# junliu111/CV-MonoSLAM

Hardware: AMD Instinct MI355X
Metric: srukf_updates_per_sec (higher is better)
Workload: dtype f64; 1 GPU; BASELINE configs[2]: 200 inverse-depth landmarks (n=1204, Na=1209, L=2419), M=N matched, fp64, one batched refactor per frame, synthetic 640x480 figure-8 sequence; landmarks=200, state_dim=1204, sequences_per_gpu=1, update_mode=batched

## Files before the change

### cv-monoslam_amd/csrc/srukf_batch.hip

```cpp

#include "srukf_ctx.h"
using namespace srukf_impl;

struct BatchPlan {
    std::vector<srukf_ctx*> cs;
    int B = 0;
    Pxy2Args* t_pxy2 = nullptr; GainArgs* t_gain = nullptr; SyrkArgs* t_syrk = nullptr; SyrkOwnArgs* t_own = nullptr; Step64Args* t_step = nullptr; ExpandArgs* t_exp = nullptr;
    hipGraph_t g1 = nullptr, g8 = nullptr; hipGraphExec_t e1 = nullptr, e8 = nullptr;
    std::vector<unsigned long long> sig;
};
struct BatchDev { BatchPlan* plans[SRUKF_BATCH_GROUPS_MAX] = {}; hipStream_t streams[SRUKF_BATCH_GROUPS_MAX] = {}; };
static thread_local std::map<int, BatchDev> g_batch_dev;
static hipStream_t batch_stream(int device, int grp)
{
    BatchDev& bd = g_batch_dev[device];
    if (!bd.streams[0]) {
        if (hipSetDevice(device) != hipSuccess) return nullptr;
        for (int q = 0; q < SRUKF_BATCH_GROUPS_MAX; q++) if (hipStreamCreateWithFlags(&bd.streams[q], hipStreamNonBlocking) != hipSuccess) bd.streams[q] = nullptr;
    }
    return bd.streams[grp];
}
static void batch_plan_drop_graphs(BatchPlan* bp)
{
    if (bp->e1) { hipGraphExecDestroy(bp->e1); bp->e1 = nullptr; }
// ... 42 lines not shown
    for (auto& kv : g_batch_dev)
        for (int grp = 0; grp < SRUKF_BATCH_GROUPS_MAX; grp++) if (kv.second.plans[grp]) { hipSetDevice(kv.first); hipStreamSynchronize(kv.second.streams[grp]); batch_plan_drop_graphs(kv.second.plans[grp]); }
}
}
static bool batch_eligible(srukf_ctx* const* cs, int B, bool ignore_canonical = false)
{
    if (B < 2 || B > 64 || !g_dbg_batch_wide.load()) return false;
    const srukf_ctx* a = cs[0];
    for (int b = 0; b < B; b++) {
        const srukf_ctx* c = cs[b];
        for (int q = 0; q < b; q++) if (cs[q] == c) return false;
        if (c->device != a->device || c->d.N != a->d.N || c->d.N < 1 || c->storage != SRUKF_STORAGE_F64 || c->w.wc0 != c->w.wm0) return false;
        if (c->red_r <= 0 || c->red_r != a->red_r || c->red_Tp != a->red_Tp || !c->shadowA || (!c->null_canonical && !ignore_canonical) || !c->nskip || !c->tail_ok) return false;
        if (c->ns_full != a->ns_full || c->ns_null != a->ns_null || c->ns_rows != a->ns_rows || c->n_pxy2_tiles != a->n_pxy2_tiles) return false;
        if (c->n_syrk_head_tiles != a->n_syrk_head_tiles || c->gplan_red.ntiles != a->gplan_red.ntiles || c->pxy2_split_b0 != a->pxy2_split_b0 || memcmp(&c->w, &a->w, sizeof c->w) != 0) return false;
        if (!c->dbg.pxy2 || !c->dbg.nullskip || !c->dbg.tail_fuse || c->dbg.fused_motion != 2 || !c->dbg.table_perm || c->profiling || c->use_graph != a->use_graph || c->debug_starve) return false;
        if (memcmp(&c->p, &a->p, sizeof c->p) != 0 || c->gplan_red.T < 16 || (size_t)c->d.np * sizeof(double) > 48 * 1024 || !rank_fused_mode()) return false;
        if (!c->odo_seq || c->seqF != a->seqF) return false;
    }
    return true;
}
static void batch_frame(const BatchPlan* bp, hipStream_t st)
{
    const srukf_ctx* c = bp->cs[0];
    const KDims& d = c->d;
    const int n = d.n, np = d.np, r = c->red_r, Tp = c->red_Tp, B = bp->B, kr = (r + 15) & ~15;
    srukf_launch_pxy2_b(st, d, bp->t_pxy2, B, c->pxy2_tiles, c->n_pxy2_tiles, kr, c->w, (d.N + 31) / 32);
    srukf_launch_gain_b(st, d, c->w, bp->t_gain, B, c->pxy2_split_b0, sqrt(c->p.epsilon));
    srukf_launch_syrk_b(st, d, bp->t_syrk, B, g_dbg_batch_xcd.load() ? c->syrk_head_tiles_b : c->syrk_head_tiles, g_dbg_batch_xcd.load() ? c->n_syrk_head_tiles_b : c->n_syrk_head_tiles, std::min(np, kr), (n + 255) / 256,
                        (n - r + SRUKF_RANK_COLS - 1) / SRUKF_RANK_COLS);
    srukf_launch_syrk_own_b(st, n, np, bp->t_own, B, 0, d.mp, kr, c->gplan_red.tiles, c->gplan_red.ntiles, Tp);
    int pb = 0;
    for (int j0 = -64; j0 + 64 < np && j0 + 64 <= 64 * Tp; j0 += 64, pb ^= 1) {
        if (!g_dbg_batch_split.load()) {
            srukf_launch_gmw_step64_b(st, n, np, j0, c->p.epsilon, bp->t_step, B, std::max(1, Tp - j0 / 64 - 1), pb);
            continue;
        }
        const int rows = Tp - j0 / 64 - 1, pair = j0 >= 0 ? (j0 / 64) & 1 : 0;
        const bool k128 = g_dbg_batch_k128.load() != 0;
        const bool first_of_pair = k128 && j0 >= 0 && pair == 0 && rows - 1 >= 1 && j0 + 128 < np && j0 + 128 <= 64 * Tp;
        const bool second_of_pair = k128 && j0 >= 64 && pair == 1 && rows >= 1;
        srukf_launch_gmw_pivslab_b(st, n, np, j0, c->p.epsilon, bp->t_step, B, pb, second_of_pair ? 1 : 0);
        if (j0 >= 0 && rows >= 1) srukf_launch_gmw_trail_b(st, np, j0, bp->t_step, B, rows, second_of_pair ? 1 : 0, first_of_pair ? 1 : second_of_pair ? 2 : 0);
    }
    srukf_launch_rank_expand_b(st, n, np, r, c->p.epsilon, bp->t_exp, B, c->w.gamma, d, c->w, c->p);
}
static int batch_capture(BatchPlan* bp, hipStream_t st, int nframes, hipGraph_t* g, hipGraphExec_t* ge)
{
    srukf_ctx* c = bp->cs[0];
    HIPCHK(c, hipStreamBeginCapture(st, hipStreamCaptureModeThreadLocal));
    for (int q = 0; q < nframes; q++) batch_frame(bp, st);
    const hipError_t launch_err = hipGetLastError();
    HIPCHK(c, hipStreamEndCapture(st, g));
    HIPCHK(c, launch_err);
    HIPCHK(c, hipGraphInstantiate(ge, *g, nullptr, nullptr, 0));
    return SRUKF_OK;
}
static int batch_run(srukf_ctx* const* cs, int B, int first, int count, double* const* dt, int grp)
{
    srukf_ctx* c0 = cs[0];
// ... 178 lines not shown
```

### cv-monoslam_amd/csrc/srukf_ctx.h

```cpp
#pragma once
#include <hip/hip_runtime.h>
#include <math.h>
#include <stdio.h>
#include <stdlib.h>
#include <string.h>
#include <string>
#include <cstddef>
#include <vector>
#include <algorithm>
#include <utility>
#include <atomic>
#include <mutex>
#include <map>
#include "srukf_launch.h"

#define SRUKF_GRAPH_FRAMES 8
#define SRUKF_MAX_TENANTS 4
#define SRUKF_NULL_ENERGY 1e-12
#ifndef SRUKF_BATCH_GROUPS_MAX
#define SRUKF_BATCH_GROUPS_MAX 4
#endif

enum KClass { KC_MOTION = 0, KC_PROJECT, KC_STATS, KC_PXY, KC_GAIN, KC_SYRK, KC_GMW_TRAIL, KC_GMW_PERSIST, KC_GMW_CHECK,
              KC_GMW_COL, KC_RANK_EXPAND, KC_PROJECT_MOTION, KC_PROJECT_TABLE, KC_PXY2, KC_MISC,
// ... 20 lines not shown
    unsigned char *patch = nullptr, *tmpl = nullptr;
};


struct srukf_switches {
    int rank_aware = 1;
    int debug_allow_mixed = 0;
    int debug_starve = 0;
    bool split_off = false;
    bool use_graph = true;
    struct DbgSwitches {
        int fused_motion = 2;
        int f32_fuse = 1;
        int table_perm = 1;
        int tail_fuse = 1;
        int head_fold = 1;
        int nullskip = 1;
        int pxy2 = 1;
        int step_fuse_export = 1;
        int view_auto = 1;
        int step_early = 2;
        int step_spin = 1;
        int step_fast = 1;
        int split_record = 0;
        int null_canon = 1;
        int split_fold = 1;
        int gain_fold = 0;
        int mixed_rank = 1;
        int mixed_null_ppm = 1;
        int mixed_bf16 = 0;
// ... 303 lines not shown
```

### cv-monoslam_amd/csrc/srukf_debug.hip

```cpp

#include "srukf_ctx.h"
using namespace srukf_impl;


namespace srukf_impl {
std::atomic<int> g_dbg_gmw_persist{1}, g_dbg_gmw_fused{1}, g_dbg_rank_fused{1}, g_dbg_rank_fold{1}, g_dbg_rank_aware{1}, g_dbg_graphs{1};
std::atomic<int> g_dbg_mem_split{1};
std::atomic<int> g_dbg_shared_tenants{2};
std::atomic<int> g_dbg_batch_wide{1}, g_dbg_batch_groups{0}, g_dbg_batch_split{1};
std::atomic<int> g_dbg_timing{0}, g_dbg_fold_head{0}, g_dbg_fold_force{0}, g_dbg_ctx_keep{24}, g_dbg_batch_xcd{1}, g_dbg_batch_k128{1};
std::atomic<int> g_dbg_head_fold_free{0};
}

static bool debug_buffer(srukf_ctx* c, const char* key, double** ptr, long long* cap)
{
    const KDims& d = c->d;
    const GmwPlan& gp = c->red_r > 0 ? c->gplan_red : c->gplan;
    double* src = nullptr; long long n = 0;
    if (!strcmp(key, "Z")) { src = c->Z; n = (long long)d.L * d.mp; }
    else if (!strcmp(key, "DZ")) { src = c->DZ; n = (long long)d.np * d.mp; }
    else if (!strcmp(key, "sigR")) { src = c->sigR; n = (long long)(d.L + 1) * 8; }
    else if (!strcmp(key, "Cmat")) { src = c->Cmat; n = (long long)d.n * 4; }
    else if (!strcmp(key, "Xr1")) { src = (double*)((char*)c->fs + offsetof(FrameScalars, Xr1)); n = 4; }
    else if (!strcmp(key, "Utp")) { src = c->Utp; n = c->Utp ? (long long)d.mp * d.np : 0; }
// ... 60 lines not shown
    for (auto& g : globals)
        if (!strcmp(key, g.k)) {
            g.v->store(!strcmp(key, "mem_split") ? value : (value ? 1 : 0));
            if (c) { hipSetDevice(c->device); step_commit_motion(c); step_invalidate(c); hipStreamSynchronize(c->stream); drop_graphs(c); if (!strcmp(key, "rank_aware")) return update_null_set(c); }
            return SRUKF_OK;
        }
    if (!c) return SRUKF_ERR_BAD_ARG;
    HIPCHK(c, hipSetDevice(c->device));
    step_commit_motion(c); step_invalidate(c);
    HIPCHK(c, hipStreamSynchronize(c->stream));
    if (!strcmp(key, "use_graph")) c->use_graph = value != 0;
    else if (!strcmp(key, "pxy2")) c->dbg.pxy2 = value ? 1 : 0;
    else if (!strcmp(key, "nullskip")) c->dbg.nullskip = value ? 1 : 0;
    else if (!strcmp(key, "head_fold")) c->dbg.head_fold = value ? 1 : 0;
    else if (!strcmp(key, "tail_fuse")) c->dbg.tail_fuse = value ? 1 : 0;
    else if (!strcmp(key, "table_perm")) c->dbg.table_perm = value ? 1 : 0;
    else if (!strcmp(key, "f32_fuse")) c->dbg.f32_fuse = value ? 1 : 0;
    else if (!strcmp(key, "split_record")) c->dbg.split_record = value ? 1 : 0;
    else if (!strcmp(key, "gain_fold")) c->dbg.gain_fold = value ? 1 : 0;
    else if (!strcmp(key, "null_canon")) c->dbg.null_canon = value ? 1 : 0;
    else if (!strcmp(key, "split_fold")) c->dbg.split_fold = value < 0 ? 0 : value > 2 ? 2 : value;
    else if (!strcmp(key, "mixed_rank")) c->dbg.mixed_rank = value ? 1 : 0;
    else if (!strcmp(key, "mixed_f64_robot")) c->dbg.mixed_f64_robot = value ? 1 : 0;
    else if (!strcmp(key, "mixed_bf16")) c->dbg.mixed_bf16 = value ? 1 : 0;
    else if (!strcmp(key, "mixed_null_ppm")) c->dbg.mixed_null_ppm = value < 0 ? 0 : value;
    else if (!strcmp(key, "step_fast")) c->dbg.step_fast = value ? 1 : 0;
    else if (!strcmp(key, "step_spin")) c->dbg.step_spin = value ? 1 : 0;
    else if (!strcmp(key, "step_early")) c->dbg.step_early = value < 0 ? 0 : value > 2 ? 2 : value;
    else if (!strcmp(key, "view_auto")) { c->dbg.view_auto = value ? 1 : 0; if (!value) { c->view_auto = false; c->view_cached = false; } }
    else if (!strcmp(key, "step_fuse_export")) c->dbg.step_fuse_export = value ? 1 : 0;
// ... 63 lines not shown
        const bool persist = plan_persists(c, gp);
        const char* k = key + 5;
        if (!strcmp(k, "T")) *value = gp.T;
        else if (!strcmp(k, "Tp")) *value = gp.Tp;
        else if (!strcmp(k, "tiles")) *value = gp.nreal;
        else if (!strcmp(k, "workers")) *value = gp.workers;
        else if (!strcmp(k, "persist")) *value = persist ? 1 : 0;
        else if (!strcmp(k, "register_form")) *value = (persist && !split_form(c, gp) && srukf_gmw_register_form(gp.T, gp.Tp, gp.ntiles, gp.workers)) ? 1 : 0;
        else if (!strcmp(k, "relay")) *value = (persist && !split_form(c, gp) && gp.relay && srukf_gmw_register_form(gp.T, gp.Tp, gp.ntiles, gp.workers)) ? 1 : 0;
        else if (!strcmp(k, "tiles_per_worker")) *value = gp.workers > 0 ? (gp.nreal + gp.workers - 1) / gp.workers : -1;
        else if (!strcmp(k, "fold")) *value = rp.form == RF_OWNERS_FOLD ? 1 : 0;
        else if (!strcmp(k, "head_fold")) *value = rp.head_fold ? 1 : 0;
        else if (!strcmp(k, "red_perm")) *value = replay_red_perm(c) ? 1 : 0;
        else if (!strcmp(k, "motion")) *value = replay_motion_mode(c);
        else if (!strcmp(k, "fuse")) *value = frame_form(c).fused_tail() ? 1 : 0;
        else if (!strcmp(k, "kept")) *value = c->red_r;
        else if (!strcmp(k, "sync_doubles")) *value = gp.sync ? srukf_gmw_sync_bytes(gp.T) / 8 : 0;
        else if (!strcmp(k, "pans_doubles")) *value = gp.pans ? (long long)srukf_gmw_panel_bytes() * gp.T / 8 : 0;
        else if (!strcmp(k, "slab_panels")) *value = c->gs_panels;
        else return SRUKF_ERR_BAD_ARG;
    }
    else return SRUKF_ERR_BAD_ARG;
    return SRUKF_OK;
}

int srukf_debug_copy(srukf_ctx* c, const char* key, double* out, long long count)
{
    if (!c || !key || !out || count < 0) return SRUKF_ERR_BAD_ARG;
    HIPCHK(c, hipSetDevice(c->device));
    HIPCHK(c, hipStreamSynchronize(c->stream));
// ... 107 lines not shown
```

### cv-monoslam_amd/csrc/srukf_launch.h

```cpp
#pragma once
#include "srukf_device.h"
#include "srukf_rank.h"

struct GmwPanel64;
struct GmwTile;


struct GmwLaunch {
    int n, ld; double eps;
    double* G; GmwPanel64* pans; double* D; double* Sout; GmwSync* sync;
    const GmwTile* tiles; int ntiles, workers;
    FrameScalars* fs;
    int Tp, krows, gate_limit, relay;
};
inline GmwLaunch gmw_normalised(GmwLaunch g)
{
    const int T = g.ld / 64;
    if (g.Tp <= 0 || g.Tp > T) g.Tp = T;
    if (g.krows <= 0 || g.krows > g.ld) g.krows = g.ld;
    return g;
}
struct GmwFused { const double* S0; const double* Ut0; int u0, u1; };

struct SyrkRider { const double* dxp; double* X; RankArgs ra; const double* xr1; };
// ... 1 lines not shown
struct GainLaunch {
    KDims d; KWeights w;
    double* Ut; const double* PxyR; const double* Si; const int* vis; const double* h;
    const double* z_seq; const double* z_cur; const int* m_seq; const int* m_cur;
    FrameScalars* fs; double* dxp; const double* Z; RankArgs ra;
    const double* Cm; double* S; const double* P1; int split_b0; const double* DZp; double sqeps; const double* sigR;
    bool fmode; const double* next_pose; double* odo_dev;
};

struct RankExpandLaunch {
    KDims d; KWeights w; srukf_params p;
    int r;
    const double* Sp; const double* D; const int* perm; const int* iperm; const double* gdiag; FrameScalars* fs; const double* X;
    double* S; double* A; double* sigR; double* Z; double* DZ;
    bool do_traj, fuse, f32round;
    const StepExport* step_export; double null_rel; unsigned int* fold_sync; int fold_words;
};

extern "C" {
void srukf_launch_landmarks_cartesian(hipStream_t st, KDims d, const double* X, const double* S, double* xyz, double* cov);
void srukf_launch_motion(hipStream_t st, KDims d, KWeights w, srukf_params p, double* X, double* S, double* sigR, double* Cmat, FrameScalars* fs, const double* odo_seq,
                         const double* odo_pair, RankArgs ra);
void srukf_launch_project_motion(hipStream_t st, KDims d, KWeights w, srukf_params p, double* X, double* S, double* sigR, double* Cm, double* Z, double* DZ, FrameScalars* fs,
                                 RankArgs ra);
void srukf_launch_project_table(hipStream_t st, KDims d, KWeights w, srukf_params p, double* X, double* S, double* sigR, double* Cm, double* Z, double* DZ, FrameScalars* fs,
                                RankArgs ra, NullSkip ns);
void srukf_launch_sigr_rows(hipStream_t st, KDims d, KWeights w, const double* X, const double* S, double* sigR, const FrameScalars* fs, const int* iperm, int rkeep);
void srukf_launch_project(hipStream_t st, KDims d, KWeights w, srukf_params p, const double* X, const double* S, const double* sigR, double* Z, double* DZ, const FrameScalars* fs);
void srukf_launch_meas_stats(hipStream_t st, KDims d, KWeights w, const double* X, const double* sigR, const double* Z, double* part, double* h, double* Si, int* vis, double* PxyR);
int srukf_meas_part_doubles(int mp);
// ... 35 lines not shown
void srukf_launch_syrk_own_b(hipStream_t st, int n, int ld, const SyrkOwnArgs* tab, int B, int u0, int u1, int krows, const GmwTile* tiles, int ntiles, int Tp);
void srukf_launch_gmw_split(hipStream_t stA, hipStream_t stB, const GmwLaunch& g, double* Wslab, double* Lslab, int starve);
void srukf_launch_gmw_split_alone(hipStream_t st, int which, const GmwLaunch& g, double* Wslab, double* Lslab);
void srukf_launch_gmw_split_fold(hipStream_t stA, hipStream_t stB, const GmwLaunch& g, double* Wslab, double* Lslab, const GmwTile* list, int nlist, const double* A, const double* Ut, int mp);
void srukf_gmw_fold_head_override(int v);
int srukf_gmw_fold_head_rows(int Tp);
int srukf_gmw_fold_head_tile(int tr, int tc, int head_rows);
int srukf_gmw_build_fold_list(int T, int Tp, short* out);
int srukf_gmw_head_rows(void);
int srukf_gmw_head_extra_diag(void);

void srukf_launch_rank_round(hipStream_t st, int ld, int r, double* A);
void srukf_launch_row_energy(hipStream_t st, int n, int ld, const double* S, double* e);
void srukf_launch_rank_diag(hipStream_t st, int n, int ld, const double* G, const int* perm, double* gdiag);
void srukf_launch_rank_expand(hipStream_t st, const RankExpandLaunch& a);
void srukf_launch_rank_expand_b(hipStream_t st, int n, int ld, int r, double eps, const ExpandArgs* tab, int B, double gamma, KDims d, KWeights w, srukf_params p);
void srukf_launch_rank_canon(hipStream_t st, int n, int ld, int r, double sq, const int* perm, double* S);
void srukf_launch_rank_shadow(hipStream_t st, int n, int ld, int r, const double* S, const int* perm, double* A);

int srukf_mixed_build_tasks_red(int np, int ue, int krows, int rows_lim, short* out_tasks, int* out_tiles, int* ntiles);
int srukf_mixed_build_tasks(int np, int ue, short* out_tasks, int* out_tiles, int* ntiles);
int srukf_mixed_krows(int r);
size_t srukf_mixed_part_bytes(int ntasks);
void srukf_launch_cvt_f32(hipStream_t st, size_t count, const double* src, float* dst);
void srukf_launch_gain_dx(hipStream_t st, int n, int np, const double* dxp, double* X, const double* xr1);
void srukf_launch_cvt_robot_cols(hipStream_t st, int n, int np, const double* S, float* S32);
void srukf_launch_syrk32(hipStream_t st, int n, int np, int ue, const float* S32, const float* U32, const void* tasks, int ntasks, const void* tiles, int ntiles, double* part,
                         double* G, FrameScalars* fs, int krows);
void srukf_launch_split_bf3(hipStream_t st, int rows, int ld, int ktot, int koff, const double* src, void* planes, size_t plane_stride);
void srukf_launch_syrk_bf3(hipStream_t st, int n, int np, int ue, int krows, int ktot, const void* planes, size_t plane_stride, const void* tasks, int ntasks, const void* tiles,
                           int ntiles, double* part, double* G, FrameScalars* fs);
// ... 20 lines not shown
```

### cv-monoslam_amd/csrc/srukf_rank.h

```cpp
#pragma once
#include <hip/hip_runtime.h>
#include "srukf_device.h"

struct RankArgs {
    double* A;
    double* Utp;
    double* gdiag;
    const int* iperm;
    const int* perm;
    int r;
    int dzperm;
    int f32round;
    int prep_next;
    int dxN;
};

struct Pxy2Args { const double* DZp; const double* A; double* P0; double* P1; MeasArgs ms; };
struct SyrkArgs { const double* S; const double* Ut; double* G; FrameScalars* fs; const double* dxp; double* X; RankArgs ra; const double* xr1; };
struct GainArgs {
    double* Ut; const double* PxyR; const double* Si; const int* vis; const double* h; const double* z_seq; const int* m_seq; FrameScalars* fs; double* dxp;
    RankArgs ra; const double* Cm; double* S; const double* P1; const double* DZp; const double* sigR; const double* Z0;
};
struct ExpandArgs {
    const double* Sp; const double* D; const int* perm; const int* iperm; const double* gdiag; FrameScalars* fs; const double* X; double* S; double* A;
    double* sigR; double* Z; double* DZ;
};

struct HeadArgs {
    const int2* tiles; int ntiles;
    int ncrit;
    const double* dxp; double* X; const double* xr1; int ndx;
    int ngd;
    int nhelp;
    RankArgs ra;
};

#define SRUKF_RANK_COLS 16
__device__ __forceinline__ double srukf_rank_colsq(const double* __restrict__ M, int ld, int rows, int a, int kl)
{
    double v = 0.0;
    for (int k = kl; k < rows; k += 20 * 16) {
        double t[20];
#pragma unroll
        for (int u = 0; u < 20; u++) t[u] = M[(size_t)min(k + 16 * u, rows - 1) * ld + a];
#pragma unroll
        for (int u = 0; u < 20; u++) v += (k + 16 * u < rows) ? t[u] * t[u] : 0.0;
    }
    return v;
}
__device__ __forceinline__ void srukf_rank_gdiag_job(int n, int ld, int mu, const RankArgs ra, unsigned long long* gmax_bits, int blk)
{
    __shared__ double cs[16][17];
// ... 13 lines not shown
```

### cv-monoslam_amd/csrc/srukf_rank.hip

```cpp
#include <hip/hip_runtime.h>
#include "srukf_device.h"
#include "srukf_rank.h"
#include "srukf_motion.h"
#include "srukf_motion_reduce.h"
#include "srukf_launch.h"

__global__ __launch_bounds__(256) void k_rank_shadow(int n, int ld, int r, const double* __restrict__ S, const int* __restrict__ perm, double* __restrict__ A)
{
    const int a = blockIdx.x;
    double* out = A + (size_t)a * ld;
    if (a >= r) { for (int b = threadIdx.x; b < ld; b += 256) out[b] = 0.0; return; }
    const double* src = S + (size_t)perm[a] * ld;
    for (int b = threadIdx.x; b < ld; b += 256) out[b] = (b >= a && b < n) ? src[perm[b]] : 0.0;
}

__global__ __launch_bounds__(256) void k_row_energy(int n, int ld, const double* __restrict__ S, double* __restrict__ e)
{
    __shared__ double red[16];
    const int k = blockIdx.x;
    double v[1] = { 0.0 };
    for (int i = k + threadIdx.x; i < n; i += 256) { const double s = S[(size_t)k * ld + i]; v[0] += s * s; }
    block_sum<1>(v, red);
    if (threadIdx.x == 0) e[k] = v[0];
}

__global__ __launch_bounds__(256) void k_rank_diag(int n, int ld, const double* __restrict__ G, const int* __restrict__ perm, double* __restrict__ gdiag)
{
    const int a = blockIdx.x * 256 + threadIdx.x;
    if (a < n) { const int j = perm[a]; gdiag[a] = G[(size_t)j * ld + j]; }
}

template <int MODE>
__device__ __forceinline__ void rank_expand_body(int n, int ld, int r, double eps, const double* __restrict__ Sp, const double* __restrict__ D,
                                                 const int* __restrict__ perm, const int* __restrict__ iperm, const double* __restrict__ gdiag,
                                                 FrameScalars* __restrict__ fs, const double* __restrict__ X, int do_traj, double* __restrict__ S,
                                                 double* __restrict__ A, double* __restrict__ sigR, double gamma,
                                                 const KDims& d, const KWeights& w,
                                                 const srukf_params& p, double* __restrict__ Z, double* __restrict__ DZ, int f32, const int bid, const StepExport& ex, const double null_rel = 0.0,
                                                 unsigned int* __restrict__ fold_sync = nullptr, const int fold_words = 0)
{
    constexpr bool PROJ = MODE == 2;
    auto rnd = [&](double v) { return f32 ? (double)(float)v : v; };
    extern __shared__ double lrow[];
    __shared__ double prow[2][8];
    __shared__ double red[16 * 3];
    const int j = bid;
    const int Na = n + 5;
    const bool table = sigR && fs->ctl_next_valid && !fs->frozen;
    auto table_rows = [&](const int i, const int sg, const double (&srow)[4], const double (&mnoise)[3], const bool isnull) {
        const MotionCtl mc = { fs->ctl[0], fs->ctl[1], fs->ctl[2], fs->ctl[3], fs->ctl[4] };
        const double xr[4] = { X[n - 4], X[n - 3], X[n - 2], X[n - 1] };
        double rr[4], c2, s2;
        if (isnull) srukf_motion_centre(mc, xr, rr, c2, s2);
        else srukf_motion_point(mc, xr, srow, mnoise, sg ? -gamma : gamma, rr, c2, s2);
        double4* o = reinterpret_cast<double4*>(sigR + (size_t)(1 + sg * Na + i) * 8);
        o[0] = make_double4(rr[0], rr[1], rr[2], rr[3]); o[1] = make_double4(c2, s2, 0.0, 0.0);
        if constexpr (PROJ) { double* q = prow[sg]; q[0] = rr[0]; q[1] = rr[1]; q[2] = rr[2]; q[3] = rr[3]; q[4] = c2; q[5] = s2; }
    };
    const double f1 = PROJ ? p.cam_f / p.cam_dx : 0.0, f2 = PROJ ? p.cam_f / p.cam_dy : 0.0;
    auto project_pair = [&](const int i, const int k, const double (&dev)[6], const double e0, const double e1, const double* r0, const double* r1, const int dzrow) {
        double base[6];
#pragma unroll
        for (int e = 0; e < 6; e++) base[e] = X[6 * k + e];
        double zp[2], zm[2];
        srukf_project_sigma(p, f1, f2, base, dev, e0, e1, gamma, r0, zp[0], zp[1]);
        srukf_project_sigma(p, f1, f2, base, dev, e0, e1, -gamma, r1, zm[0], zm[1]);
        *reinterpret_cast<double2*>(Z + (size_t)(1 + i) * d.mp + 2 * k) = make_double2(zp[0], zp[1]);
        *reinterpret_cast<double2*>(Z + (size_t)(1 + Na + i) * d.mp + 2 * k) = make_double2(zm[0], zm[1]);
        if (dzrow >= 0) *reinterpret_cast<double2*>(DZ + (size_t)dzrow * d.mp + 2 * k) = make_double2(zp[0] - zm[0], zp[1] - zm[1]);
    };
    if constexpr (PROJ) {
        const int nchk = (n - r + SRUKF_RANK_COLS - 1) / SRUKF_RANK_COLS;
        if (j > n + nchk) {
            if (!table) return;
            const int q = j - n - nchk - 1;
            if (threadIdx.x < 2) {
                const double zero4[4] = { 0, 0, 0, 0 };
                double mnoise[3] = { 0, 0, 0 };
                if (q < 3) mnoise[q] = fs->ctl[5 + q];
                table_rows(n + q, threadIdx.x, zero4, mnoise, false);
            }
            __syncthreads();
            const double zero6[6] = { 0, 0, 0, 0, 0, 0 };
            const double e0 = (q == 3) ? p.sigma_measure : 0.0, e1 = (q == 4) ? p.sigma_measure : 0.0;
            for (int k = threadIdx.x; k < d.N; k += 256) project_pair(n + q, k, zero6, e0, e1, prow[0], prow[1], -1);
            return;
        }
    }
    if (j == n) {
        if (fold_sync) {
            const int base = (fold_words + FOLD_FLAG_STRIDE - 1) / FOLD_FLAG_STRIDE * FOLD_FLAG_STRIDE;
            for (int q = threadIdx.x; q < fold_words; q += 256) fold_sync[q] = 0u;
            if (threadIdx.x < 2 + SRUKF_STAT_GROUPS) fold_sync[base + FOLD_FLAG_STRIDE * threadIdx.x] = 0u;
        }
        if (table && threadIdx.x < (PROJ ? 1 : 11)) {
            const double zero4[4] = { 0, 0, 0, 0 };
            if (threadIdx.x == 0) {
                const MotionCtl mc = { fs->ctl[0], fs->ctl[1], fs->ctl[2], fs->ctl[3], fs->ctl[4] };
                const double xr[4] = { X[n - 4], X[n - 3], X[n - 2], X[n - 1] };
                double s0[4], c0s, s0s;
// ... 76 lines not shown
    if (j > n) {
        const int a = r + SRUKF_RANK_COLS * (j - n - 1) + (threadIdx.x & 15), kl = threadIdx.x >> 4;
        __shared__ double cs[16][17];
        cs[kl][threadIdx.x & 15] = (a < n) ? srukf_rank_colsq(Sp, ld, r, a, kl) : 0.0;
        __syncthreads();
        if (threadIdx.x < 16 && a < n) {
            double t = 0.0;
            for (int q = 0; q < 16; q++) t += cs[q][threadIdx.x];
            if (gdiag[a] - t > 1e-12 + null_rel * fabs(gdiag[a])) { atomicAdd(&fs->clamp_rows, 1); atomicMin(&fs->clamp_first, perm[a]); }
        }
        return;
    }
    const int a = j;
    const int jj = perm[a];
    double* out = S + (size_t)jj * ld;
    if (table && threadIdx.x < 2) {
        double srow[4] = { 0, 0, 0, 0 };
        const double zero3[3] = { 0, 0, 0 };
        if (a < r) {
#pragma unroll
            for (int e = 0; e < 4; e++) srow[e] = (r - 4 + e >= a) ? rnd(Sp[(size_t)a * ld + (r - 4 + e)]) : 0.0;
        }
        table_rows(jj, threadIdx.x, srow, zero3, a >= r);
    }
    if (a >= r) {
        if constexpr (PROJ) {
            if (table) {
                __syncthreads();
                if (threadIdx.x < 2) {
                    const int k = jj / 6, sg = threadIdx.x;
                    double dev[6], base[6];
#pragma unroll
                    for (int e = 0; e < 6; e++) { dev[e] = (6 * k + e == jj) ? rnd(sqrt(eps)) : 0.0; base[e] = X[6 * k + e]; }
                    double ox, oy;
                    srukf_project_sigma(p, f1, f2, base, dev, 0.0, 0.0, sg ? -gamma : gamma, prow[sg], ox, oy);
                    *reinterpret_cast<double2*>(Z + (size_t)(1 + sg * Na + jj) * d.mp + 2 * k) = make_double2(ox, oy);
                    const double pox = __shfl_xor(ox, 1), poy = __shfl_xor(oy, 1);
                    if (sg == 0) *reinterpret_cast<double2*>(DZ + (size_t)a * d.mp + 2 * k) = make_double2(ox - pox, oy - poy);
                }
            }
        }
        if (sigR && fs->const_rows_ok) return;
// ... 25 lines not shown
    }
    mx = wave_max(mx);
    if ((threadIdx.x & 63) == 0) red[threadIdx.x >> 6] = mx;
    __syncthreads();
    if (threadIdx.x == 0) {
        mx = fmax(fmax(red[0], red[1]), fmax(red[2], red[3]));
        const double gamma = __longlong_as_double((long long)fs->gmax_bits);
        const double xi = __longlong_as_double((long long)fs->ximax_bits);
        const double nu = fmax(1.0, sqrt((double)n * n - 1.0));
        const double beta2 = fmax(fmax(gamma, xi / nu), 1e-15);
        const double dj = D[a];
        const double th = mx * sqrt(dj);
        if (th * th / beta2 > dj) { atomicAdd(&fs->clamp_rows, 1); atomicMin(&fs->clamp_first, jj); }
    }
    if constexpr (PROJ) {
        if (table) {
            for (int k = threadIdx.x; k < d.N; k += 256) {
                double dev[6];
#pragma unroll
                for (int e = 0; e < 6; e++) { const int col = 6 * k + e; dev[e] = (col >= jj) ? lrow[iperm[col]] : 0.0; }
                project_pair(jj, k, dev, 0.0, 0.0, prow[0], prow[1], a);
            }
        }
    }
}

template <int MODE>
__global__ __launch_bounds__(256) void k_rank_expand(int n, int ld, int r, double eps, const double* __restrict__ Sp, const double* __restrict__ D,
                                                     const int* __restrict__ perm, const int* __restrict__ iperm, const double* __restrict__ gdiag,
                                                     FrameScalars* __restrict__ fs, const double* __restrict__ X, int do_traj, double* __restrict__ S,
                                                     double* __restrict__ A, double* __restrict__ sigR, double gamma,
                                                     KDims d, KWeights w,
                                                     srukf_params p, double* __restrict__ Z, double* __restrict__ DZ, int f32, StepExport ex, double null_rel,
                                                     unsigned int* __restrict__ fold_sync, int fold_words)
{
    const int extra = (int)gridDim.x - n;
    const int bid = (int)blockIdx.x < extra ? n + (int)blockIdx.x : (int)blockIdx.x - extra;
    rank_expand_body<MODE>(n, ld, r, eps, Sp, D, perm, iperm, gdiag, fs, X, do_traj, S, A, sigR, gamma, d, w, p, Z, DZ, f32, bid, ex, null_rel, fold_sync, fold_words);
    if (!ex.dst) return;
    const int ncount = extra + r;
    if ((int)blockIdx.x >= ncount) return;
    __shared__ int last;
    asm volatile("s_waitcnt vmcnt(0)" ::: "memory");
    __syncthreads();
    if (threadIdx.x == 0) {
        const int g = (int)blockIdx.x & 63, gsize = (ncount - g + 63) >> 6, groups = ncount < 64 ? ncount : 64;
        int* c1 = ex.cnt + 64 * g;
        last = 0;
        if (__hip_atomic_fetch_add(c1, 1, __ATOMIC_RELAXED, __HIP_MEMORY_SCOPE_AGENT) == gsize - 1) {
            __hip_atomic_store(c1, 0, __ATOMIC_RELAXED, __HIP_MEMORY_SCOPE_AGENT);
            if (__hip_atomic_fetch_add(&fs->export_cnt, 1, __ATOMIC_RELAXED, __HIP_MEMORY_SCOPE_AGENT) == groups - 1) {
                __hip_atomic_store(&fs->export_cnt, 0, __ATOMIC_RELAXED, __HIP_MEMORY_SCOPE_AGENT);
                last = 1;
// ... 3 lines not shown
    __syncthreads();
    if (!last) return;
    const unsigned long long* fw = (const unsigned long long*)fs;
    for (int i = threadIdx.x; i < ex.nfs; i += 256) ex.dst[i] = __hip_atomic_load(fw + i, __ATOMIC_RELAXED, __HIP_MEMORY_SCOPE_AGENT);
    if (threadIdx.x < 20) ((double*)(ex.dst + ex.nfs))[threadIdx.x] = ld_dev(ex.view + threadIdx.x);
    __threadfence_system();
    __syncthreads();
    if (threadIdx.x == 0) {
        if (ex.set && __hip_atomic_load(&fs->clamp_rows, __ATOMIC_RELAXED, __HIP_MEMORY_SCOPE_AGENT) == 0) {
            for (int e = 0; e < 6; e++) ex.odo[e] = ex.poses[e];
            srukf_step_scalars(fs, ex.odo, 1, ex.a, false);
        }
        if (ex.flag) __hip_atomic_store(ex.flag, ex.seq, __ATOMIC_RELEASE, __HIP_MEMORY_SCOPE_SYSTEM);
    }
}
__global__ __launch_bounds__(256) void k_rank_expand_b(int n, int ld, int r, double eps, const ExpandArgs* __restrict__ tab, int per, double gamma, KDims d, KWeights w, srukf_params p)
{
    const int f = (int)blockIdx.x / per, bid = (int)blockIdx.x - f * per;
    const ExpandArgs a = tab[f];
    rank_expand_body<2>(n, ld, r, eps, a.Sp, a.D, a.perm, a.iperm, a.gdiag, a.fs, a.X, 1, a.S, a.A, a.sigR, gamma, d, w, p, a.Z, a.DZ, 0, bid, StepExport{});
}

__global__ __launch_bounds__(256) void k_rank_round(int ld, double* __restrict__ A)
{
    double* row = A + (size_t)blockIdx.x * ld;
    for (int b = blockIdx.x + threadIdx.x; b < ld; b += 256) row[b] = (double)(float)row[b];
}

extern "C" {
void srukf_launch_rank_round(hipStream_t st, int ld, int r, double* A)
{
    hipLaunchKernelGGL(k_rank_round, dim3(r), dim3(256), 0, st, ld, A);
}
void srukf_launch_row_energy(hipStream_t st, int n, int ld, const double* S, double* e)
{
    hipLaunchKernelGGL(k_row_energy, dim3(n), dim3(256), 0, st, n, ld, S, e);
}
void srukf_launch_rank_diag(hipStream_t st, int n, int ld, const double* G, const int* perm, double* gdiag)
{
    hipLaunchKernelGGL(k_rank_diag, dim3((n + 255) / 256), dim3(256), 0, st, n, ld, G, perm, gdiag);
}
void srukf_launch_rank_expand(hipStream_t st, const RankExpandLaunch& a)
{
    const int n = a.d.n, ld = a.d.np, r = a.r, do_traj = a.do_traj ? 1 : 0;
    const bool fuse = a.fuse;
    const double eps = a.p.epsilon;
    const StepExport ex = (a.step_export && fuse) ? *a.step_export : StepExport{};
    const int nchk = (n - r + SRUKF_RANK_COLS - 1) / SRUKF_RANK_COLS;
    const dim3 grid(n + 1 + nchk + (fuse ? 5 : 0));
    if (fuse) hipLaunchKernelGGL(k_rank_expand<2>, grid, dim3(256), sizeof(double) * (size_t)ld, st, n, ld, r, eps, a.Sp, a.D, a.perm, a.iperm, a.gdiag, a.fs, a.X, do_traj, a.S, a.A, a.sigR, a.w.gamma, a.d, a.w, a.p, a.Z, a.DZ, a.f32round ? 1 : 0, ex, a.null_rel, a.fold_sync, a.fold_words);
    else hipLaunchKernelGGL(k_rank_expand<0>, grid, dim3(256), 0, st, n, ld, r, eps, a.Sp, a.D, a.perm, a.iperm, a.gdiag, a.fs, a.X, do_traj, a.S, a.A, a.sigR, a.w.gamma, a.d, a.w, a.p, a.Z, a.DZ, 0, StepExport{}, a.null_rel, a.fold_sync, a.fold_words);
}
void srukf_launch_rank_expand_b(hipStream_t st, int n, int ld, int r, double eps, const ExpandArgs* tab, int B, double gamma, KDims d, KWeights w, srukf_params p)
{
    const int nchk = (n - r + SRUKF_RANK_COLS - 1) / SRUKF_RANK_COLS;
    const int per = n + 1 + nchk + 5;
    hipLaunchKernelGGL(k_rank_expand_b, dim3(per * B), dim3(256), sizeof(double) * (size_t)ld, st, n, ld, r, eps, tab, per, gamma, d, w, p);
}
__global__ __launch_bounds__(256) void k_rank_canon(int n, int ld, int r, double sq, const int* __restrict__ perm, double* __restrict__ S)
{
    const int k = perm[r + blockIdx.x];
    if (k < 0 || k >= n) return;
    for (int c = threadIdx.x; c < ld; c += 256) S[(size_t)k * ld + c] = (c == k) ? sq : 0.0;
}
void srukf_launch_rank_canon(hipStream_t st, int n, int ld, int r, double sq, const int* perm, double* S)
{
    if (n - r > 0) hipLaunchKernelGGL(k_rank_canon, dim3(n - r), dim3(256), 0, st, n, ld, r, sq, perm, S);
}
void srukf_launch_rank_shadow(hipStream_t st, int n, int ld, int r, const double* S, const int* perm, double* A)
{
    hipLaunchKernelGGL(k_rank_shadow, dim3(ld), dim3(256), 0, st, n, ld, r, S, perm, A);
}
// ... 2 lines not shown
```

### cv-monoslam_amd/csrc/srukf_replay.hip

```cpp

#include "srukf_ctx.h"
using namespace srukf_impl;

__global__ void k_refactor_reset(int np, unsigned long long* theta_bits, FrameScalars* fs, int reset_stats)
{
    const int i = blockIdx.x * blockDim.x + threadIdx.x;
    if (i < np) theta_bits[i] = 0ull;
    if (i == 0 && reset_stats) { fs->gmax_bits = 0ull; fs->ximax_bits = 0ull; }
}

__global__ void k_set_seq(FrameScalars* fs, const double* odo_seq, int seqF, double a1, double a2, double a3, double a4)
{
    fs->odo_seq = odo_seq; fs->seqF = seqF;
    fs->a[0] = a1; fs->a[1] = a2; fs->a[2] = a3; fs->a[3] = a4;
}

__global__ void k_set_frame(FrameScalars* fs, int frame, int clear_clamp)
{
    fs->frame = frame;
    srukf_prepare_control(fs);
    fs->stat_count = 0;
    fs->const_rows_ok = 0; fs->const_rows_pending = 0;
    for (int q = 0; q < SRUKF_STAT_GROUPS; q++) fs->stat_cnt[q] = 0;
    fs->traj_base = nullptr;
// ... 192 lines not shown
int gate_limit(const srukf_ctx* c) { return c->gmw_shared == 1 ? c->shared_tenants : 0; }

static void rank_expand(srukf_ctx* c, const RefactorRequest& rq, FrameForm ff)
{
    const int np = c->d.np;
    const bool frame_tail = rq.kind == RefactorRequest::FRAME_TAIL, table = ff.robot_table, fuse = ff.fused_tail();
    const bool f32s = c->storage != SRUKF_STORAGE_F64;
    const bool f32fuse = storage_f32_like(c) && fuse && table && frame_tail;
    const bool f32 = f32s && !f32fuse;
    const bool tt = table && frame_tail && !f32;
    const bool exports = c->step_export.dst && tt && fuse;
    srukf_launch_rank_expand(c->stream, RankExpandLaunch{
        .d = c->d, .w = c->w, .p = c->p, .r = c->red_r,
        .Sp = c->G, .D = c->D, .perm = c->red_perm, .iperm = c->red_iperm, .gdiag = c->gdiag, .fs = c->fs, .X = c->X,
        .S = c->S, .A = c->shadowA, .sigR = tt ? c->sigR : nullptr, .Z = c->Z, .DZ = c->DZ,
        .do_traj = frame_tail && !f32, .fuse = tt && fuse, .f32round = f32fuse,
        .step_export = exports ? &c->step_export : nullptr,
        .null_rel = c->storage == SRUKF_STORAGE_F32_MIXED ? 1e-6 * c->dbg.mixed_null_ppm : 0.0,
        .fold_sync = (tt && fuse) ? c->fold_sync : nullptr, .fold_words = c->fold_sync ? 4 * (c->d.mp / 64) * (c->d.np / 64) : 0 });
    c->step_export_attached = exports;
    if (f32) {
        quantize_state(c);
        srukf_launch_rank_round(c->stream, np, c->red_r, c->shadowA);
        if (frame_tail) srukf_launch_traj(c->stream, c->d, c->X, c->S, c->fs, nullptr, 1);
    }
}

static int fold_tiles_pct(const srukf_ctx* c) { return c->gmw_shared == 1 ? 200 : 106; }

static bool replay_red_fused(const srukf_ctx* c)
{
// ... 833 lines not shown
```

Measured before the change: 5595 frames/s.

## Pack null-row sigma projections into dense lane groups in rank expand

Adds a tail_pack mode, on by default, to the fused rank-expand kernel. Null-space rows (a >= r) no longer run a per-block two-thread projection; their ± sigma projections go to extra packed blocks where each lane handles one (row, sign) pair. Kept rows project per (landmark, sign) lane instead of per landmark. The ragged remainder of kept rows can be spilled into extra blocks when occupancy allows. The aim is to cut idle lanes and serialized tail work in the projection phase. The cost is more blocks, recomputed motion centres per lane, and shuffle-based DZ differencing that relies on adjacent-lane pairing.

```diff
diff --git a/cv-monoslam_amd/csrc/srukf_batch.hip b/cv-monoslam_amd/csrc/srukf_batch.hip
--- a/cv-monoslam_amd/csrc/srukf_batch.hip
+++ b/cv-monoslam_amd/csrc/srukf_batch.hip
@@ -80,7 +80,7 @@
         if (c->red_r <= 0 || c->red_r != a->red_r || c->red_Tp != a->red_Tp || !c->shadowA || (!c->null_canonical && !ignore_canonical) || !c->nskip || !c->tail_ok) return false;
         if (c->ns_full != a->ns_full || c->ns_null != a->ns_null || c->ns_rows != a->ns_rows || c->n_pxy2_tiles != a->n_pxy2_tiles) return false;
         if (c->n_syrk_head_tiles != a->n_syrk_head_tiles || c->gplan_red.ntiles != a->gplan_red.ntiles || c->pxy2_split_b0 != a->pxy2_split_b0 || memcmp(&c->w, &a->w, sizeof c->w) != 0) return false;
-        if (!c->dbg.pxy2 || !c->dbg.nullskip || !c->dbg.tail_fuse || c->dbg.fused_motion != 2 || !c->dbg.table_perm || c->profiling || c->use_graph != a->use_graph || c->debug_starve) return false;
+        if (!c->dbg.pxy2 || !c->dbg.nullskip || !c->dbg.tail_fuse || c->dbg.fused_motion != 2 || !c->dbg.table_perm || c->dbg.tail_pack != a->dbg.tail_pack || c->profiling || c->use_graph != a->use_graph || c->debug_starve) return false;
         if (memcmp(&c->p, &a->p, sizeof c->p) != 0 || c->gplan_red.T < 16 || (size_t)c->d.np * sizeof(double) > 48 * 1024 || !rank_fused_mode()) return false;
         if (!c->odo_seq || c->seqF != a->seqF) return false;
     }
@@ -109,7 +109,7 @@
         srukf_launch_gmw_pivslab_b(st, n, np, j0, c->p.epsilon, bp->t_step, B, pb, second_of_pair ? 1 : 0);
         if (j0 >= 0 && rows >= 1) srukf_launch_gmw_trail_b(st, np, j0, bp->t_step, B, rows, second_of_pair ? 1 : 0, first_of_pair ? 1 : second_of_pair ? 2 : 0);
     }
-    srukf_launch_rank_expand_b(st, n, np, r, c->p.epsilon, bp->t_exp, B, c->w.gamma, d, c->w, c->p);
+    srukf_launch_rank_expand_b(st, n, np, r, c->p.epsilon, bp->t_exp, B, c->w.gamma, d, c->w, c->p, c->dbg.tail_pack != 0);
 }
 static int batch_capture(BatchPlan* bp, hipStream_t st, int nframes, hipGraph_t* g, hipGraphExec_t* ge)
 {
diff --git a/cv-monoslam_amd/csrc/srukf_ctx.h b/cv-monoslam_amd/csrc/srukf_ctx.h
--- a/cv-monoslam_amd/csrc/srukf_ctx.h
+++ b/cv-monoslam_amd/csrc/srukf_ctx.h
@@ -58,6 +58,7 @@
         int f32_fuse = 1;
         int table_perm = 1;
         int tail_fuse = 1;
+        int tail_pack = 1;
         int head_fold = 1;
         int nullskip = 1;
         int pxy2 = 1;
diff --git a/cv-monoslam_amd/csrc/srukf_debug.hip b/cv-monoslam_amd/csrc/srukf_debug.hip
--- a/cv-monoslam_amd/csrc/srukf_debug.hip
+++ b/cv-monoslam_amd/csrc/srukf_debug.hip
@@ -98,6 +98,7 @@
     else if (!strcmp(key, "nullskip")) c->dbg.nullskip = value ? 1 : 0;
     else if (!strcmp(key, "head_fold")) c->dbg.head_fold = value ? 1 : 0;
     else if (!strcmp(key, "tail_fuse")) c->dbg.tail_fuse = value ? 1 : 0;
+    else if (!strcmp(key, "tail_pack")) { c->dbg.tail_pack = value ? 1 : 0; batch_drop_all_graphs(); }
     else if (!strcmp(key, "table_perm")) c->dbg.table_perm = value ? 1 : 0;
     else if (!strcmp(key, "f32_fuse")) c->dbg.f32_fuse = value ? 1 : 0;
     else if (!strcmp(key, "split_record")) c->dbg.split_record = value ? 1 : 0;
@@ -191,6 +192,7 @@
         else if (!strcmp(k, "red_perm")) *value = replay_red_perm(c) ? 1 : 0;
         else if (!strcmp(k, "motion")) *value = replay_motion_mode(c);
         else if (!strcmp(k, "fuse")) *value = frame_form(c).fused_tail() ? 1 : 0;
+        else if (!strcmp(k, "tail_pack")) *value = (frame_form(c).fused_tail() && c->dbg.tail_pack) ? 1 : 0;
         else if (!strcmp(k, "kept")) *value = c->red_r;
         else if (!strcmp(k, "sync_doubles")) *value = gp.sync ? srukf_gmw_sync_bytes(gp.T) / 8 : 0;
         else if (!strcmp(k, "pans_doubles")) *value = gp.pans ? (long long)srukf_gmw_panel_bytes() * gp.T / 8 : 0;
diff --git a/cv-monoslam_amd/csrc/srukf_launch.h b/cv-monoslam_amd/csrc/srukf_launch.h
--- a/cv-monoslam_amd/csrc/srukf_launch.h
+++ b/cv-monoslam_amd/csrc/srukf_launch.h
@@ -39,6 +39,7 @@
     const double* Sp; const double* D; const int* perm; const int* iperm; const double* gdiag; FrameScalars* fs; const double* X;
     double* S; double* A; double* sigR; double* Z; double* DZ;
     bool do_traj, fuse, f32round;
+    bool tail_pack; int cus;
     const StepExport* step_export; double null_rel; unsigned int* fold_sync; int fold_words;
 };
 
@@ -104,7 +105,7 @@
 void srukf_launch_row_energy(hipStream_t st, int n, int ld, const double* S, double* e);
 void srukf_launch_rank_diag(hipStream_t st, int n, int ld, const double* G, const int* perm, double* gdiag);
 void srukf_launch_rank_expand(hipStream_t st, const RankExpandLaunch& a);
-void srukf_launch_rank_expand_b(hipStream_t st, int n, int ld, int r, double eps, const ExpandArgs* tab, int B, double gamma, KDims d, KWeights w, srukf_params p);
+void srukf_launch_rank_expand_b(hipStream_t st, int n, int ld, int r, double eps, const ExpandArgs* tab, int B, double gamma, KDims d, KWeights w, srukf_params p, bool tail_pack);
 void srukf_launch_rank_canon(hipStream_t st, int n, int ld, int r, double sq, const int* perm, double* S);
 void srukf_launch_rank_shadow(hipStream_t st, int n, int ld, int r, const double* S, const int* perm, double* A);
 
diff --git a/cv-monoslam_amd/csrc/srukf_rank.h b/cv-monoslam_amd/csrc/srukf_rank.h
--- a/cv-monoslam_amd/csrc/srukf_rank.h
+++ b/cv-monoslam_amd/csrc/srukf_rank.h
@@ -36,6 +36,9 @@
 };
 
 #define SRUKF_RANK_COLS 16
+__host__ __device__ inline int srukf_rank_pack_groups(int n, int r) { return (2 * (n - r) + 255) / 256; }
+__host__ __device__ inline int srukf_rank_pack_main(int N) { return 2 * N < 256 ? 2 * N : (2 * N / 256) * 256; }
+__host__ __device__ inline int srukf_rank_pack_left(int N, int r) { return (int)(((long long)r * (2 * N - srukf_rank_pack_main(N)) + 255) / 256); }
 __device__ __forceinline__ double srukf_rank_colsq(const double* __restrict__ M, int ld, int rows, int a, int kl)
 {
     double v = 0.0;
diff --git a/cv-monoslam_amd/csrc/srukf_rank.hip b/cv-monoslam_amd/csrc/srukf_rank.hip
--- a/cv-monoslam_amd/csrc/srukf_rank.hip
+++ b/cv-monoslam_amd/csrc/srukf_rank.hip
@@ -1,4 +1,5 @@
 #include <hip/hip_runtime.h>
+#include <atomic>
 #include "srukf_device.h"
 #include "srukf_rank.h"
 #include "srukf_motion.h"
@@ -37,9 +38,13 @@
                                                  double* __restrict__ A, double* __restrict__ sigR, double gamma,
                                                  const KDims& d, const KWeights& w,
                                                  const srukf_params& p, double* __restrict__ Z, double* __restrict__ DZ, int f32, const int bid, const StepExport& ex, const double null_rel = 0.0,
-                                                 unsigned int* __restrict__ fold_sync = nullptr, const int fold_words = 0)
+                                                 unsigned int* __restrict__ fold_sync = nullptr, const int fold_words = 0, const int pack_on = 0)
 {
     constexpr bool PROJ = MODE == 2;
+    const bool pack = PROJ && pack_on;
+    const int nleft = pack ? pack_on - 1 : 0;
+    const int Mmain = nleft > 0 ? srukf_rank_pack_main(d.N) : 2 * d.N;
+    const bool lanes_all = pack && (2 * d.N + 255) / 256 < 2 * ((d.N + 255) / 256), lanes_row = lanes_all || nleft > 0;
     auto rnd = [&](double v) { return f32 ? (double)(float)v : v; };
     extern __shared__ double lrow[];
     __shared__ double prow[2][8];
@@ -69,8 +74,62 @@
         *reinterpret_cast<double2*>(Z + (size_t)(1 + Na + i) * d.mp + 2 * k) = make_double2(zm[0], zm[1]);
         if (dzrow >= 0) *reinterpret_cast<double2*>(DZ + (size_t)dzrow * d.mp + 2 * k) = make_double2(zp[0] - zm[0], zp[1] - zm[1]);
     };
+    auto project_one = [&](const int i, const int k, const int sg, const double (&dev)[6], const double e0, const double e1, const double* rb, const int dzrow) {
+        double base[6];
+#pragma unroll
+        for (int e = 0; e < 6; e++) base[e] = X[6 * k + e];
+        double ox, oy;
+        srukf_project_sigma(p, f1, f2, base, dev, e0, e1, sg ? -gamma : gamma, rb, ox, oy);
+        *reinterpret_cast<double2*>(Z + (size_t)(1 + sg * Na + i) * d.mp + 2 * k) = make_double2(ox, oy);
+        if (dzrow >= 0) {
+            const double pox = __shfl_xor(ox, 1), poy = __shfl_xor(oy, 1);
+            if (sg == 0) *reinterpret_cast<double2*>(DZ + (size_t)dzrow * d.mp + 2 * k) = make_double2(ox - pox, oy - poy);
+        }
+    };
     if constexpr (PROJ) {
         const int nchk = (n - r + SRUKF_RANK_COLS - 1) / SRUKF_RANK_COLS;
+        if (pack && j > n + nchk + 5 + nleft) {
+            if (!table) return;
+            const int t = 256 * (j - n - nchk - 6 - nleft) + (int)threadIdx.x, a = r + (t >> 1), sg = t & 1;
+            if (a >= n) return;
+            const int jj = perm[a], k = jj / 6;
+            const MotionCtl mc = { fs->ctl[0], fs->ctl[1], fs->ctl[2], fs->ctl[3], fs->ctl[4] };
+            const double xr[4] = { X[n - 4], X[n - 3], X[n - 2], X[n - 1] };
+            double rr[4], c2, s2;
+            srukf_motion_centre(mc, xr, rr, c2, s2);
+            double4* o = reinterpret_cast<double4*>(sigR + (size_t)(1 + sg * Na + jj) * 8);
+            o[0] = make_double4(rr[0], rr[1], rr[2], rr[3]); o[1] = make_double4(c2, s2, 0.0, 0.0);
+            const double rb[6] = { rr[0], rr[1], rr[2], rr[3], c2, s2 };
+            double dev[6];
+#pragma unroll
+            for (int e = 0; e < 6; e++) dev[e] = (6 * k + e == jj) ? rnd(sqrt(eps)) : 0.0;
+            project_one(jj, k, sg, dev, 0.0, 0.0, rb, a);
+            return;
+        }
+        if (pack && j > n + nchk + 5) {
+            if (!table) return;
+            const int per = 2 * d.N - Mmain;
+            const int fl = 256 * (j - n - nchk - 6) + (int)threadIdx.x, a = fl / per, t = Mmain + fl - a * per;
+            if (a >= r) return;
+            const int jj = perm[a], k = t >> 1, sg = t & 1;
+            const double* src = Sp + (size_t)a * ld;
+            const MotionCtl mc = { fs->ctl[0], fs->ctl[1], fs->ctl[2], fs->ctl[3], fs->ctl[4] };
+            const double xr[4] = { X[n - 4], X[n - 3], X[n - 2], X[n - 1] };
+            const double zero3[3] = { 0, 0, 0 };
+            double srow[4], rr[4], c2, s2;
+#pragma unroll
+            for (int e = 0; e < 4; e++) srow[e] = (r - 4 + e >= a) ? rnd(src[r - 4 + e]) : 0.0;
+            srukf_motion_point(mc, xr, srow, zero3, sg ? -gamma : gamma, rr, c2, s2);
+            const double rb[6] = { rr[0], rr[1], rr[2], rr[3], c2, s2 };
+            double dev[6];
+#pragma unroll
+            for (int e = 0; e < 6; e++) {
+                const int col = 6 * k + e, b = iperm[col];
+                dev[e] = (col >= jj && b >= a) ? rnd(src[b]) : 0.0;
+            }
+            project_one(jj, k, sg, dev, 0.0, 0.0, rb, a);
+            return;
+        }
         if (j > n + nchk) {
             if (!table) return;
             const int q = j - n - nchk - 1;
@@ -83,7 +142,8 @@
             __syncthreads();
             const double zero6[6] = { 0, 0, 0, 0, 0, 0 };
             const double e0 = (q == 3) ? p.sigma_measure : 0.0, e1 = (q == 4) ? p.sigma_measure : 0.0;
-            for (int k = threadIdx.x; k < d.N; k += 256) project_pair(n + q, k, zero6, e0, e1, prow[0], prow[1], -1);
+            if (lanes_all) for (int t = threadIdx.x; t < 2 * d.N; t += 256) project_one(n + q, t >> 1, t & 1, zero6, e0, e1, prow[t & 1], -1);
+            else for (int k = threadIdx.x; k < d.N; k += 256) project_pair(n + q, k, zero6, e0, e1, prow[0], prow[1], -1);
             return;
         }
     }
@@ -190,7 +250,7 @@
     const int a = j;
     const int jj = perm[a];
     double* out = S + (size_t)jj * ld;
-    if (table && threadIdx.x < 2) {
+    if (table && threadIdx.x < 2 && !(pack && a >= r)) {
         double srow[4] = { 0, 0, 0, 0 };
         const double zero3[3] = { 0, 0, 0 };
         if (a < r) {
@@ -201,7 +261,7 @@
     }
     if (a >= r) {
         if constexpr (PROJ) {
-            if (table) {
+            if (table && !pack) {
                 __syncthreads();
                 if (threadIdx.x < 2) {
                     const int k = jj / 6, sg = threadIdx.x;
@@ -257,7 +317,15 @@
         if (th * th / beta2 > dj) { atomicAdd(&fs->clamp_rows, 1); atomicMin(&fs->clamp_first, jj); }
     }
     if constexpr (PROJ) {
-        if (table) {
+        if (table && lanes_row) {
+            for (int t = threadIdx.x; t < Mmain; t += 256) {
+                const int k = t >> 1;
+                double dev[6];
+#pragma unroll
+                for (int e = 0; e < 6; e++) { const int col = 6 * k + e; dev[e] = (col >= jj) ? lrow[iperm[col]] : 0.0; }
+                project_one(jj, k, t & 1, dev, 0.0, 0.0, prow[t & 1], a);
+            }
+        } else if (table) {
             for (int k = threadIdx.x; k < d.N; k += 256) {
                 double dev[6];
 #pragma unroll
@@ -275,11 +343,11 @@
                                                      double* __restrict__ A, double* __restrict__ sigR, double gamma,
                                                      KDims d, KWeights w,
                                                      srukf_params p, double* __restrict__ Z, double* __restrict__ DZ, int f32, StepExport ex, double null_rel,
-                                                     unsigned int* __restrict__ fold_sync, int fold_words)
+                                                     unsigned int* __restrict__ fold_sync, int fold_words, int pack)
 {
     const int extra = (int)gridDim.x - n;
     const int bid = (int)blockIdx.x < extra ? n + (int)blockIdx.x : (int)blockIdx.x - extra;
-    rank_expand_body<MODE>(n, ld, r, eps, Sp, D, perm, iperm, gdiag, fs, X, do_traj, S, A, sigR, gamma, d, w, p, Z, DZ, f32, bid, ex, null_rel, fold_sync, fold_words);
+    rank_expand_body<MODE>(n, ld, r, eps, Sp, D, perm, iperm, gdiag, fs, X, do_traj, S, A, sigR, gamma, d, w, p, Z, DZ, f32, bid, ex, null_rel, fold_sync, fold_words, pack);
     if (!ex.dst) return;
     const int ncount = extra + r;
     if ((int)blockIdx.x >= ncount) return;
@@ -313,11 +381,11 @@
         if (ex.flag) __hip_atomic_store(ex.flag, ex.seq, __ATOMIC_RELEASE, __HIP_MEMORY_SCOPE_SYSTEM);
     }
 }
-__global__ __launch_bounds__(256) void k_rank_expand_b(int n, int ld, int r, double eps, const ExpandArgs* __restrict__ tab, int per, double gamma, KDims d, KWeights w, srukf_params p)
+__global__ __launch_bounds__(256) void k_rank_expand_b(int n, int ld, int r, double eps, const ExpandArgs* __restrict__ tab, int per, double gamma, KDims d, KWeights w, srukf_params p, int pack)
 {
     const int f = (int)blockIdx.x / per, bid = (int)blockIdx.x - f * per;
     const ExpandArgs a = tab[f];
-    rank_expand_body<2>(n, ld, r, eps, a.Sp, a.D, a.perm, a.iperm, a.gdiag, a.fs, a.X, 1, a.S, a.A, a.sigR, gamma, d, w, p, a.Z, a.DZ, 0, bid, StepExport{});
+    rank_expand_body<2>(n, ld, r, eps, a.Sp, a.D, a.perm, a.iperm, a.gdiag, a.fs, a.X, 1, a.S, a.A, a.sigR, gamma, d, w, p, a.Z, a.DZ, 0, bid, StepExport{}, 0.0, nullptr, 0, pack);
 }
 
 __global__ __launch_bounds__(256) void k_rank_round(int ld, double* __restrict__ A)
@@ -346,15 +414,23 @@
     const double eps = a.p.epsilon;
     const StepExport ex = (a.step_export && fuse) ? *a.step_export : StepExport{};
     const int nchk = (n - r + SRUKF_RANK_COLS - 1) / SRUKF_RANK_COLS;
-    const dim3 grid(n + 1 + nchk + (fuse ? 5 : 0));
-    if (fuse) hipLaunchKernelGGL(k_rank_expand<2>, grid, dim3(256), sizeof(double) * (size_t)ld, st, n, ld, r, eps, a.Sp, a.D, a.perm, a.iperm, a.gdiag, a.fs, a.X, do_traj, a.S, a.A, a.sigR, a.w.gamma, a.d, a.w, a.p, a.Z, a.DZ, a.f32round ? 1 : 0, ex, a.null_rel, a.fold_sync, a.fold_words);
-    else hipLaunchKernelGGL(k_rank_expand<0>, grid, dim3(256), 0, st, n, ld, r, eps, a.Sp, a.D, a.perm, a.iperm, a.gdiag, a.fs, a.X, do_traj, a.S, a.A, a.sigR, a.w.gamma, a.d, a.w, a.p, a.Z, a.DZ, 0, StepExport{}, a.null_rel, a.fold_sync, a.fold_words);
-}
-void srukf_launch_rank_expand_b(hipStream_t st, int n, int ld, int r, double eps, const ExpandArgs* tab, int B, double gamma, KDims d, KWeights w, srukf_params p)
+    int pack = 0;
+    if (fuse && a.tail_pack) {
+        static std::atomic<int> slots_per_cu{0};
+        int slots = slots_per_cu.load();
+        if (slots == 0 && hipOccupancyMaxActiveBlocksPerMultiprocessor(&slots, k_rank_expand<2>, 256, sizeof(double) * (size_t)ld) == hipSuccess) slots_per_cu.store(slots);
+        const int nleft = srukf_rank_pack_left(a.d.N, r);
+        pack = 1 + ((nleft > 0 && 1 + nchk + 5 + nleft + r <= slots * a.cus) ? nleft : 0);
+    }
+    const dim3 grid(n + 1 + nchk + (fuse ? 5 : 0) + (pack ? pack - 1 + srukf_rank_pack_groups(n, r) : 0));
+    if (fuse) hipLaunchKernelGGL(k_rank_expand<2>, grid, dim3(256), sizeof(double) * (size_t)ld, st, n, ld, r, eps, a.Sp, a.D, a.perm, a.iperm, a.gdiag, a.fs, a.X, do_traj, a.S, a.A, a.sigR, a.w.gamma, a.d, a.w, a.p, a.Z, a.DZ, a.f32round ? 1 : 0, ex, a.null_rel, a.fold_sync, a.fold_words, pack);
+    else hipLaunchKernelGGL(k_rank_expand<0>, grid, dim3(256), 0, st, n, ld, r, eps, a.Sp, a.D, a.perm, a.iperm, a.gdiag, a.fs, a.X, do_traj, a.S, a.A, a.sigR, a.w.gamma, a.d, a.w, a.p, a.Z, a.DZ, 0, StepExport{}, a.null_rel, a.fold_sync, a.fold_words, 0);
+}
+void srukf_launch_rank_expand_b(hipStream_t st, int n, int ld, int r, double eps, const ExpandArgs* tab, int B, double gamma, KDims d, KWeights w, srukf_params p, bool tail_pack)
 {
     const int nchk = (n - r + SRUKF_RANK_COLS - 1) / SRUKF_RANK_COLS;
-    const int per = n + 1 + nchk + 5;
-    hipLaunchKernelGGL(k_rank_expand_b, dim3(per * B), dim3(256), sizeof(double) * (size_t)ld, st, n, ld, r, eps, tab, per, gamma, d, w, p);
+    const int per = n + 1 + nchk + 5 + (tail_pack ? srukf_rank_pack_groups(n, r) : 0);
+    hipLaunchKernelGGL(k_rank_expand_b, dim3(per * B), dim3(256), sizeof(double) * (size_t)ld, st, n, ld, r, eps, tab, per, gamma, d, w, p, tail_pack ? 1 : 0);
 }
 __global__ __launch_bounds__(256) void k_rank_canon(int n, int ld, int r, double sq, const int* __restrict__ perm, double* __restrict__ S)
 {
diff --git a/cv-monoslam_amd/csrc/srukf_replay.hip b/cv-monoslam_amd/csrc/srukf_replay.hip
--- a/cv-monoslam_amd/csrc/srukf_replay.hip
+++ b/cv-monoslam_amd/csrc/srukf_replay.hip
@@ -230,7 +230,7 @@
         .d = c->d, .w = c->w, .p = c->p, .r = c->red_r,
         .Sp = c->G, .D = c->D, .perm = c->red_perm, .iperm = c->red_iperm, .gdiag = c->gdiag, .fs = c->fs, .X = c->X,
         .S = c->S, .A = c->shadowA, .sigR = tt ? c->sigR : nullptr, .Z = c->Z, .DZ = c->DZ,
-        .do_traj = frame_tail && !f32, .fuse = tt && fuse, .f32round = f32fuse,
+        .do_traj = frame_tail && !f32, .fuse = tt && fuse, .f32round = f32fuse, .tail_pack = c->dbg.tail_pack != 0, .cus = c->gplan_red.cus,
         .step_export = exports ? &c->step_export : nullptr,
         .null_rel = c->storage == SRUKF_STORAGE_F32_MIXED ? 1e-6 * c->dbg.mixed_null_ppm : 0.0,
         .fold_sync = (tt && fuse) ? c->fold_sync : nullptr, .fold_words = c->fold_sync ? 4 * (c->d.mp / 64) * (c->d.np / 64) : 0 });
```

Measured after the change: 5646 frames/s, median of 6. No clear change (+0.9%).
